# aws-samples/sagemaker-distributed-training-pytorch-kr

Measured on AMD Instinct MI355X. Metric: tokens/sec (whole node) GPT-2 345M pretrain, higher is better.
Workload: dtype bf16; 1 GPU; model=gpt2-345m (24L h1024 16A, vocab 50304), global_batch=64, seq_len=1024, micro_batch=64, grad_accum=1, parallelism=tp1pp1dp1, layout=baseline, tp=1, pp=1, dp=1, flash_attn=True, recompute=none, gemm_autotune=preloaded, comm_stream_priority=high, optimizer_overlap=False, mlp_gelu_fusion=gemm_tn epilogues (fc1 bias+GeLU fwd, fc2 dgrad+GeLU bwd)

## Files before the change

sagemaker-distributed-training-pytorch-kr_amd/csrc/bindings.cpp:

```cpp
#include <torch/extension.h>
#include <c10/hip/HIPStream.h>
#include <c10/hip/HIPGuard.h>

#include "kernels/launchers.h"

namespace {

using torch::Tensor;
using OptT = std::optional<Tensor>;

hipStream_t cur_stream() { return c10::hip::getCurrentHIPStream().stream(); }

int dcode(const Tensor& t) {
  switch (t.scalar_type()) {
    case at::kFloat: return 0;
    case at::kBFloat16: return 1;
    case at::kHalf: return 2;
    default: TORCH_CHECK(false, "smdt_amd: unsupported dtype ", t.scalar_type());
  }
}

void check(hipError_t e, const char* what) {
  TORCH_CHECK(e == hipSuccess, "smdt_amd kernel '", what, "' failed: ", hipGetErrorString(e));
}
// ... 408 lines not shown
  check(smdt_gemm_mx((int)out_dtype, a.scalar_type() == at::kFloat8_e5m2 ? 1 : 0, a.data_ptr(), sa.data_ptr(),
                     b.data_ptr(), sb.data_ptr(), out.data_ptr(), optr(bias), M, N, K, (int)max_blocks, cur_stream()),
        "gemm_mx");
  return out;
}

void fp8_update_scales(Tensor scale, Tensor hist, Tensor amax, Tensor fmt_max, int64_t margin, bool use_max) {
  need_contig(scale, "scale");
  need_contig(hist, "amax_history");
  need_contig(amax, "amax");
  need_contig(fmt_max, "fmt_max");
  TORCH_CHECK(scale.dim() == 1 && hist.dim() == 2 && amax.dim() == 1 && fmt_max.dim() == 1,
              "fp8_update_scales: scale [T], amax_history [T, H], amax [T], fmt_max [T]");
  const int64_t T = scale.size(0), H = hist.size(1);
  TORCH_CHECK(T >= 1 && H >= 1 && hist.size(0) == T && amax.size(0) == T && fmt_max.size(0) == T,
              "fp8_update_scales: table sizes do not match");
  for (const Tensor* t : {&scale, &hist, &amax, &fmt_max})
    TORCH_CHECK(t->scalar_type() == at::kFloat && t->device() == scale.device(), "fp8_update_scales: fp32 tables "
                "on one device");
  TORCH_CHECK(margin >= 0 && margin <= 64, "fp8_update_scales: margin out of range");
  check(smdt_fp8_update_scales(scale.data_ptr<float>(), hist.data_ptr<float>(), amax.data_ptr<float>(),
                               fmt_max.data_ptr<float>(), T, H, (int)margin, use_max ? 1 : 0, cur_stream()),
        "fp8_update_scales");
}

Tensor transpose2d(Tensor x) {
  need_contig(x, "x");
  TORCH_CHECK(x.dim() == 2, "transpose2d: x must be 2-D");
  TORCH_CHECK(x.scalar_type() == at::kBFloat16 || x.scalar_type() == at::kHalf, "transpose2d: bf16 / fp16 only");
  TORCH_CHECK(x.size(0) % 8 == 0 && x.size(1) % 8 == 0, "transpose2d: both dims must be multiples of 8");
  auto out = torch::empty({x.size(1), x.size(0)}, x.options());
  check(smdt_transpose16(x.data_ptr(), out.data_ptr(), x.size(0), x.size(1), cur_stream()), "transpose2d");
  return out;
}

void paced_copy(Tensor recv, Tensor send, int64_t blocks, int64_t ns) {
  need_contig(recv, "recv");
  need_contig(send, "send");
  TORCH_CHECK(recv.is_cuda() && send.is_cuda(), "paced_copy: CUDA tensors");
  const int64_t nb = send.numel() * send.element_size();
  TORCH_CHECK(nb == recv.numel() * recv.element_size() && nb % 16 == 0, "paced_copy: equal sizes, multiple of 16 B");
  TORCH_CHECK((uintptr_t)send.data_ptr() % 16 == 0 && (uintptr_t)recv.data_ptr() % 16 == 0, "paced_copy: 16-B aligned");
  check(smdt_paced_copy(send.data_ptr(), recv.data_ptr(), nb, (int)blocks, ns, cur_stream()), "paced_copy");
}

void rope_(Tensor x, Tensor cos_t, Tensor sin_t, int64_t rot, int64_t pos_div, int64_t pos_mod,
           bool backward) {
  need_cuda(x, "x");
  TORCH_CHECK(x.dim() == 3 && x.stride(2) == 1, "rope: x must be [ntok, nh, d] with unit last stride");
  need_contig(cos_t, "cos");
  need_contig(sin_t, "sin");
  TORCH_CHECK(cos_t.scalar_type() == at::kFloat && sin_t.scalar_type() == at::kFloat, "rope: fp32 tables");
  TORCH_CHECK(rot <= x.size(2) && rot % 16 == 0 && cos_t.size(-1) == rot / 2, "rope: rotary dim mismatch");
  TORCH_CHECK(x.stride(0) % 8 == 0 && x.stride(1) % 8 == 0, "rope: strides must keep 16-byte alignment");
  check(smdt_rope(dcode(x), x.data_ptr(), x.size(0), (int)x.size(1), x.stride(0), x.stride(1),
                  (int)rot, cos_t.data_ptr<float>(), sin_t.data_ptr<float>(), (int)pos_div,
                  (int)pos_mod, backward ? 1 : 0, cur_stream()),
        "rope");
}

bool gemm_tn_supported(Tensor a, Tensor b) {
  if (!a.is_cuda() || !b.is_cuda() || a.dim() != 2 || b.dim() != 2 || !a.is_contiguous() || !b.is_contiguous()) return false;
  if ((a.scalar_type() != at::kBFloat16 && a.scalar_type() != at::kHalf) || b.scalar_type() != a.scalar_type()) return false;
  if (a.size(1) != b.size(1)) return false;
  if (reinterpret_cast<uintptr_t>(a.data_ptr()) % 16 || reinterpret_cast<uintptr_t>(b.data_ptr()) % 16) return false;
  return smdt_gemm_tn_supported(a.size(0), b.size(0), a.size(1)) != 0;
// ... 625 lines not shown
  check(smdt_relay_epoch_bump(s.data(), (int)s.size(), (int)rank, (int)nranks_local, (uint32_t)n, cur_stream()),
        "relay_epoch_bump");
}

}

void register_blaslt(pybind11::module_& m);

PYBIND11_MODULE(TORCH_EXTENSION_NAME, m) {
  m.doc() = "smdt_amd gfx950 (MI355X) HIP kernel library";
  register_blaslt(m);
  using pybind11::arg;
  m.def("layernorm_fwd", &layernorm_fwd, arg("x"), arg("res"), arg("bias"), arg("gamma"), arg("beta"),
        arg("eps"), arg("p_drop"), arg("seed"), arg("offset"), arg("rms"), arg("want_s"),
        arg("out_y") = pybind11::none(), arg("x2") = pybind11::none());
  m.def("layernorm_bwd", &layernorm_bwd, arg("dy"), arg("ds_in"), arg("s"), arg("gamma"), arg("mean"),
        arg("rstd"), arg("p_drop"), arg("seed"), arg("offset"), arg("rms"), arg("want_dx"), arg("want_dbias"),
        arg("dgamma_acc") = pybind11::none(), arg("dbeta_acc") = pybind11::none(),
        arg("dbias_acc") = pybind11::none(), arg("out_dx") = pybind11::none(), arg("dy2") = pybind11::none());
  m.def("bias_act_fwd", &bias_act_fwd);
  m.def("bias_act_bwd", &bias_act_bwd, arg("dy"), arg("x"), arg("bias"), arg("act"), arg("want_dbias"),
        arg("dbias_acc") = pybind11::none());
  m.def("swiglu_fwd", &swiglu_fwd);
  m.def("swiglu_bwd", &swiglu_bwd);
  m.def("softmax_fwd", &softmax_fwd);
  m.def("softmax_bwd", &softmax_bwd);
  m.def("adam", &adam);
  m.def("sumsq", &sumsq);
  m.def("clip_coef", &clip_coef);
  m.def("scale_", &scale_);
  m.def("cast_", &cast_);
  m.def("rope_", &rope_);
  m.def("transpose2d", &transpose2d);
  m.def("fp8_quantize", &fp8_quantize);
  m.def("fp8_update_scales", &fp8_update_scales);
  m.def("mx_quantize", &mx_quantize, arg("x"), arg("fmt"), arg("rows") = true, arg("cols") = false);
  m.def("gemm_mx", &gemm_mx, arg("a"), arg("sa"), arg("b"), arg("sb"), arg("bias") = pybind11::none(),
        arg("out_dtype") = 1, arg("max_blocks") = 0);
  m.def("gemm_mx_supported", &gemm_mx_supported);
  m.def("paced_copy", &paced_copy);
  m.def("gather_rows", &gather_rows);
  m.def("aug_depthwise", &aug_depthwise);
  m.def("aug_median3", &aug_median3);
  m.def("bias_grad", &bias_grad);
  m.def("gemm_tn_supported", &gemm_tn_supported, arg("a"), arg("b"));
  m.def("gemm_tn", &gemm_tn, arg("a"), arg("b"), arg("epi") = 0, arg("bias") = pybind11::none(),
        arg("out") = pybind11::none(), arg("out2") = pybind11::none(), arg("max_blocks") = 0,
        arg("var") = 0, arg("aux") = pybind11::none());
  m.def("wgrad_mfma", &wgrad_mfma, arg("main_grad"), arg("dy"), arg("x"), arg("max_splits") = 0);
  m.def("wgrad_grouped", &wgrad_grouped, arg("main_grads"), arg("dys"), arg("xs"),
        arg("biases") = std::vector<Tensor>{}, arg("overwrite") = std::vector<bool>{}, arg("cus") = 0,
        arg("mranges") = std::vector<Tensor>{}, arg("experts") = std::vector<int64_t>{});
  m.def("moe_rows", [](int64_t T, int64_t E) { return smdt_moe_rows(T, E); });
  m.def("gemm_tn_shape_supported", [](int64_t M, int64_t N, int64_t K) { return smdt_gemm_tn_supported(M, N, K) != 0; });
  m.def("moe_route", &moe_route);
  m.def("moe_route_into", &moe_route_into);
  m.def("ptr_table", &ptr_table);
  m.def("gemm_tn_grouped", &gemm_tn_grouped, arg("a"), arg("btab"), arg("n"), arg("tile_expert"), arg("epi") = 0,
        arg("biastab") = pybind11::none(), arg("aux") = pybind11::none(), arg("sums") = false,
        arg("max_blocks") = 0);
  m.def("wgrad_fp8_grouped", &wgrad_fp8_grouped, arg("main_grads"), arg("dys"), arg("xs"), arg("inv_dys"),
        arg("inv_xs"), arg("overwrite") = std::vector<bool>{}, arg("cus") = 0);
  m.def("wgrad_fp8_supported", &wgrad_fp8_supported);
  m.def("ce_stats", &ce_stats);
  m.def("set_rng_step", &set_rng_step);
  m.def("adam_capturable", &adam_capturable);
// ... 45 lines not shown
```

sagemaker-distributed-training-pytorch-kr_amd/csrc/kernels/launchers.h:

```cpp
#pragma once
#include <hip/hip_runtime.h>
#include <stdint.h>

extern "C" {

int smdt_ln_bwd_nblocks(int64_t rows, int H);
hipError_t smdt_layernorm_fwd(int dtype, int wdtype, const void* x, const void* res,
                              const void* bias, const void* gamma, const void* beta, void* y,
                              void* s_out, float* mean, float* rstd, int64_t rows, int H,
                              float eps, float p_drop, uint64_t seed, uint64_t offset, int rms,
                              const void* x2, hipStream_t st);
hipError_t smdt_layernorm_bwd(int dtype, int wdtype, const void* dy, const void* ds_in,
                              const void* s, const void* gamma, const float* mean,
                              const float* rstd, void* ds_out, void* dx_out, float* partials,
                              int nblocks, float* dgamma, float* dbeta, float* dbias,
                              int64_t rows, int H, float p_drop, uint64_t seed, uint64_t offset,
                              int rms, int acc_mask, const void* dy2, hipStream_t st);

int smdt_bias_act_slices(int64_t rows, int N);
hipError_t smdt_bias_act_fwd(int dtype, int act, const void* x, const void* bias, void* y,
                             int64_t rows, int N, hipStream_t st);
hipError_t smdt_bias_act_bwd(int dtype, int act, const void* dy, const void* x, const void* bias,
                             void* dx, float* partials, float* dbias, int64_t rows, int N,
                             int accumulate, hipStream_t st);
// ... 4 lines not shown
hipError_t smdt_swiglu_fwd(int dtype, const void* x, void* y, int64_t rows, int F,
                           hipStream_t st);
hipError_t smdt_swiglu_bwd(int dtype, const void* dy, const void* x, void* dx, int64_t rows,
                           int F, hipStream_t st);

hipError_t smdt_softmax_fwd(int dtype, int mode, const void* x, const uint8_t* mask, void* y,
                            int64_t rows, int sq, int sk, int heads, float scale,
                            hipStream_t st);
hipError_t smdt_softmax_bwd(int dtype, int mode, const void* dy, const void* y, void* dx,
                            int64_t rows, int sq, int sk, float scale, hipStream_t st);

extern "C" void smdt_set_rng_step(uint32_t* counter);
extern "C" uint32_t* smdt_rng_step();

hipError_t smdt_adam(float* master, const float* grad, float* m, float* v, void* model_out,
                     int model_dtype, int64_t n, float lr, float beta1, float beta2, float eps,
                     float wd, float bc1, float bc2, int adamw, const float* grad_mul,
                     const int* found_inf, const float* hyper, hipStream_t st);
int smdt_sumsq_nblocks(int64_t n);
hipError_t smdt_sumsq(int dtype, const void* x, int64_t n, float* partial, int nblocks,
                      float* out, int* found_inf, hipStream_t st);
hipError_t smdt_clip_coef(const float* sumsq, float max_norm, float inv_scale, float* mul_out,
                          float* norm_out, hipStream_t st);
hipError_t smdt_scale(int dtype, void* x, int64_t n, const float* mul, float cmul,
                      hipStream_t st);
hipError_t smdt_cast(int in_dtype, int out_dtype, const void* x, void* y, int64_t n,
                     int accumulate, hipStream_t st);

hipError_t smdt_rope(int dtype, void* x, int64_t ntok, int nh, int64_t tok_stride,
                     int64_t head_stride, int rot, const float* cos_t, const float* sin_t,
                     int pos_div, int pos_mod, int backward, hipStream_t st);

hipError_t smdt_transpose16(const void* in, void* out, int64_t R, int64_t C, hipStream_t st);
hipError_t smdt_fp8_quantize(const void* x, void* q, void* qt, const float* scale, float* amax, int64_t M,
                             int64_t K, int dtype, int bf8, hipStream_t st);
hipError_t smdt_fp8_update_scales(float* scale, float* hist, float* amax, const float* fmt_max, int64_t T,
                                  int64_t H, int margin, int use_max, hipStream_t st);
hipError_t smdt_mx_quantize(const void* x, void* q, void* s, void* qt, void* st, int64_t R, int64_t C, int dtype,
                            int bf8, hipStream_t st_);
int smdt_gemm_mx_supported(int64_t M, int64_t N, int64_t K);
hipError_t smdt_gemm_mx(int dtype, int a_bf8, const void* a, const void* sa, const void* b, const void* sb, void* c,
                        const void* bias, int64_t M, int64_t N, int64_t K, int max_blocks, hipStream_t st);
hipError_t smdt_paced_copy(const void* src, void* dst, int64_t nbytes, int blocks, int64_t ns, hipStream_t st);
hipError_t smdt_gather_rows(const void* src, const int64_t* map, void* dst, int64_t nrows, int64_t nsrc,
                            int64_t row_bytes, hipStream_t st);

hipError_t smdt_ce_stats(int dtype, const void* logits, const int64_t* target, int64_t rows,
                         int V, int Vvalid, int64_t vstart, float* row_max, float* row_sumexp,
                         float* row_tgt, hipStream_t st);
hipError_t smdt_ce_bwd(int dtype, const void* logits, const int64_t* target, const float* gmax,
                       const float* gsum, const float* dloss, void* dlogits, int64_t rows, int V,
                       int Vvalid, int64_t vstart, int64_t ignore_index, hipStream_t st);
hipError_t smdt_ce_fused(int dtype, void* logits, const int64_t* target, float* loss, int64_t rows,
                         int V, int Vvalid, int64_t ignore_index, int local, int64_t vstart, hipStream_t st);

hipError_t smdt_aug_depthwise(const float* x, const float* k, float* y, int N, int C, int H, int W, int ks,
                              hipStream_t st);
hipError_t smdt_aug_median3(const float* x, float* y, int planes, int H, int W, hipStream_t st);

hipError_t smdt_flash_fwd(int dtype, const void* q, const void* k, const void* v, void* o,
                          float* lse, int B, int H, int Hkv, int S, int D, int64_t q_sb,
                          int64_t q_ss, int64_t q_sh, int64_t k_sb, int64_t k_ss, int64_t k_sh,
                          int64_t v_sb, int64_t v_ss, int64_t v_sh, int64_t o_sb, int64_t o_ss,
                          int64_t o_sh, float scale, int causal, float dropout_p, uint64_t seed,
                          uint64_t offset, hipStream_t st);
hipError_t smdt_flash_bwd(int dtype, const void* q, const void* k, const void* v, const void* o,
// ... 110 lines not shown
```

sagemaker-distributed-training-pytorch-kr_amd/csrc/kernels/transpose.hip:

```cpp
#include "common.h"
#include "launchers.h"

namespace smdt {

constexpr int kTT = 64;

__global__ __launch_bounds__(256) void transpose16_kernel(const uint16_t* __restrict__ in,
                                                          uint16_t* __restrict__ out, int R, int C) {
  __shared__ uint16_t t[kTT][kTT + 2];
  const int r0 = blockIdx.x * kTT, c0 = blockIdx.y * kTT;
#pragma unroll
  for (int k = 0; k < 2; ++k) {
    const int v = threadIdx.x + k * 256;
    const int rr = v >> 3, cv = (v & 7) * 8;
    const int r = r0 + rr, c = c0 + cv;
    if (r < R && c < C) {
      const u16x8 x = __builtin_nontemporal_load(reinterpret_cast<const u16x8*>(in + (int64_t)r * C + c));
#pragma unroll
      for (int j = 0; j < 8; ++j) t[rr][cv + j] = x[j];
    }
  }
  __syncthreads();
#pragma unroll
  for (int k = 0; k < 2; ++k) {
    const int v = threadIdx.x + k * 256;
    const int cc = v >> 3, rv = (v & 7) * 8;
    const int c = c0 + cc, r = r0 + rv;
    if (c < C && r < R) {
      u16x8 y;
#pragma unroll
      for (int j = 0; j < 8; ++j) y[j] = t[rv + j][cc];
      *reinterpret_cast<u16x8*>(out + (int64_t)c * R + r) = y;
    }
  }
}

__global__ __launch_bounds__(512) void gather_rows_kernel(const uint8_t* __restrict__ src,
                                                          const int64_t* __restrict__ map,
                                                          uint8_t* __restrict__ dst, int64_t nrows,
                                                          int64_t nsrc, int64_t rb) {
  const int64_t chunks = (rb + 1023) / 1024;
  const int64_t item = (int64_t)blockIdx.x * 8 + (threadIdx.x >> 6);
  if (item >= nrows * chunks) return;
  const int64_t r = item / chunks;
  const int64_t off = (item - r * chunks) * 1024 + (int64_t)(threadIdx.x & 63) * 16;
  if (off >= rb) return;
  const int64_t s = map[r];
  u16x8 v = {};
  if (s >= 0 && s < nsrc) v = __builtin_nontemporal_load(reinterpret_cast<const u16x8*>(src + s * rb + off));
  *reinterpret_cast<u16x8*>(dst + r * rb + off) = v;
}

}

using namespace smdt;

extern "C" hipError_t smdt_gather_rows(const void* src, const int64_t* map, void* dst, int64_t nrows,
                                       int64_t nsrc, int64_t row_bytes, hipStream_t st) {
  if (nrows <= 0) return hipSuccess;
  if (row_bytes <= 0 || row_bytes % 16 != 0) return hipErrorInvalidValue;
  const int64_t items = nrows * ((row_bytes + 1023) / 1024);
  const int64_t blocks = (items + 7) / 8;
  if (blocks > 0x7FFFFFFF) return hipErrorInvalidValue;
  hipLaunchKernelGGL(gather_rows_kernel, dim3((unsigned)blocks), dim3(512), 0, st, (const uint8_t*)src, map,
                     (uint8_t*)dst, nrows, nsrc, row_bytes);
  return hipGetLastError();
}

extern "C" hipError_t smdt_transpose16(const void* in, void* out, int64_t R, int64_t C, hipStream_t st) {
  if (R <= 0 || C <= 0 || R % 8 != 0 || C % 8 != 0 || R > (1 << 30) || C > (1 << 30))
    return hipErrorInvalidValue;
  const int64_t gx = (R + kTT - 1) / kTT, gy = (C + kTT - 1) / kTT;
  if (gy > 65535) return hipErrorInvalidValue;
  hipLaunchKernelGGL(transpose16_kernel, dim3((unsigned)gx, (unsigned)gy), dim3(256), 0, st,
                     (const uint16_t*)in, (uint16_t*)out, (int)R, (int)C);
  return hipGetLastError();
}
```

sagemaker-distributed-training-pytorch-kr_amd/models/transformer.py:

```python
from __future__ import annotations

import math
import os
from dataclasses import dataclass, field
from typing import Optional

import torch
import torch.nn as nn
import torch.nn.functional as F

from ..ops import _ext
from ..ops import functional as SF
from ..parallel import state as ps
from ..parallel import tensor_parallel as tp
from ..parallel.random import checkpoint as rng_checkpoint, get_rng


@dataclass
class TransformerConfig:
    num_layers: int = 24
    hidden_size: int = 1024
    num_attention_heads: int = 16
    num_query_groups: Optional[int] = None
    ffn_hidden_size: Optional[int] = None
# ... 505 lines not shown
            cfg.params_dtype, device, None, 0, 1))
        self.router_bias = nn.Parameter(torch.zeros(e, dtype=cfg.params_dtype, device=device))
        self.experts = nn.ModuleList(ParallelMLP(cfg, layer_number, device, key=f"layers.{layer_number}.experts.{i}")
                                     for i in range(e))
        self._tabs = None

    def route(self, flat):
        prob = torch.softmax(F.linear(flat, self.router, self.router_bias).float(), dim=-1)
        return prob.max(dim=-1)

    def _grouped_check(self, flat):
        cfg = self.cfg
        why = None
        if ps.get_state().tp > 1:
            why = "tensor parallel size 1"
        elif cfg.activation != "gelu":
            why = f"the gelu activation (got {cfg.activation})"
        elif not cfg.add_bias_linear:
            why = "linear biases (--disable-bias-linear is set)"
        elif cfg.fp8:
            why = "16-bit experts (fp8 is set)"
        kern = _ext.use_kernels(flat)
        if why is None and kern:
            T, h, f, E = flat.shape[0], cfg.hidden_size, cfg.ffn_hidden_size, len(self.experts)
            R = SF.moe_rows(T, E)
            C = _ext.ext()
            probe = self.experts[0]
            if flat.dtype not in (torch.bfloat16, torch.float16) or probe.fc1.weight.dtype != flat.dtype:
                why = f"bf16 or fp16 activations and weights (got {flat.dtype} / {probe.fc1.weight.dtype})"
            elif not (C.gemm_tn_shape_supported(R, f, h) and C.gemm_tn_shape_supported(R, h, f)):
                why = (f"gemm_tn shapes: hidden {h} and ffn {f} multiples of 256 (rows {R})")
            elif torch.is_grad_enabled() and any(
                    getattr(p, "main_grad", None) is None or p.main_grad.dtype != torch.float32
                    or isinstance(getattr(type(p), "main_grad", None), property)
                    for ex in self.experts for p in (ex.fc1.weight, ex.fc1.bias, ex.fc2.weight, ex.fc2.bias)):
                why = "a plain fp32 main_grad on every expert weight and bias (a DDP wrapper with fp32 gradients)"
        if why is not None:
            raise RuntimeError(f"--moe-grouped-gemm needs {why}")
        return kern

    def _forward_grouped(self, x):
        s, b, h = x.shape
        flat = x.reshape(s * b, h)
        kern = self._grouped_check(flat)
        logits = F.linear(flat, self.router, self.router_bias)
        route = SF.moe_route(logits)
        self.last_counts = route[6]
        top_p = torch.softmax(logits.float(), dim=-1).gather(1, route[1].long().unsqueeze(1)).squeeze(1)
        ex = self.experts
        w1, b1 = [e.fc1.weight for e in ex], [e.fc1.bias for e in ex]
        w2, b2 = [e.fc2.weight for e in ex], [e.fc2.bias for e in ex]
        tabs = None
        if kern:
            key = tuple(p.data_ptr() for p in w1 + b1 + w2 + b2)
            if self._tabs is None or self._tabs[0] != key:
                self._tabs = (key, (SF.moe_pointer_tables(w1, b1), SF.moe_pointer_tables(w2, b2)))
            tabs = self._tabs[1]
        out = tp.GroupedSwitchExperts.apply(flat, top_p, route, tabs, len(ex), *w1, *b1, *w2, *b2)
        return out.view(s, b, h), None

    def forward(self, x):
        if self.cfg.moe_grouped_gemm:
            return self._forward_grouped(x)
        s, b, h = x.shape
        flat = x.reshape(s * b, h)
        top_p, top_e = self.route(flat)
        order = torch.argsort(top_e, stable=True)
# ... 179 lines not shown
```

sagemaker-distributed-training-pytorch-kr_amd/optim/optimizer.py:

```python
from __future__ import annotations

import math
import os
from typing import Optional

import torch
import torch.distributed as dist

from ..comm import health as _health
from ..comm import stats as _cs
from ..ops import _ext
from ..parallel import state as ps
from ..parallel.distributed import DistributedDataParallel
from ..parallel import tensor_parallel as _tp


class DynamicLossScaler:

    def __init__(self, initial_scale=2.0 ** 32, min_scale=1.0, growth_factor=2.0, backoff_factor=0.5,
                 growth_interval=1000, hysteresis=2, device=None):
        self.scale = torch.tensor([float(initial_scale)], dtype=torch.float32, device=device)
        self.min_scale = float(min_scale)
        self.growth_factor, self.backoff_factor = growth_factor, backoff_factor
        self.growth_interval = int(growth_interval)
# ... 211 lines not shown
        if gr.dtype != torch.float32:
            gr = gr.float()
        if use_k:
            model_out = None if self.param_is_fp32 else ddp.param_data[s:e]
            host_out = None
            if model_out is not None and not model_out.is_cuda:
                host_out, model_out = model_out, torch.empty(n, dtype=model_out.dtype, device=mst.device)
            if self.capturable:
                _ext.ext().adam_capturable(mst, gr, m, v, model_out, self._hyp, self.beta1, self.beta2,
                                           self.eps, wd, self.adamw, mul, self.found_inf)
            else:
                _ext.ext().adam(mst, gr, m, v, model_out, self.lr, self.beta1, self.beta2, self.eps, wd, t,
                                self.adamw, mul, self.found_inf)
            if host_out is not None:
                host_out.copy_(model_out)
            if self.param_is_fp32:
                ddp.param_data[s:e].copy_(mst)
        else:
            ok = (self.found_inf == 0).float()
            gg = torch.where(self.found_inf == 0, gr * mul, torch.zeros_like(gr))
            if not self.adamw and wd:
                gg = gg + wd * mst
            m.mul_(1 - (1 - self.beta1) * ok).add_(gg * ((1 - self.beta1) * ok))
            v.mul_(1 - (1 - self.beta2) * ok).add_(gg * gg * ((1 - self.beta2) * ok))
            denom = v.sqrt() / math.sqrt(bc2) + self.eps
            upd = (m / bc1) / denom
            if self.adamw and wd:
                upd = upd + wd * mst
            mst.sub_(self.lr * upd * ok)
            ddp.param_data[s:e].copy_(mst.to(ddp.param_data.dtype))

    def _step_overlapped(self, g, mul, t):
        ddp = self.ddp
        cur = torch.cuda.current_stream(self.device)
        if getattr(self, "_opt_stream", None) is None:
            self._opt_stream = torch.cuda.Stream(device=self.device)
        side = self._opt_stream
        side.wait_stream(cur)
        delay = int(os.environ.get("SMDT_OPT_STREAM_DELAY", "0"))
        with torch.cuda.stream(side):
            for i in ddp.opt_bucket_order:
                if delay:
                    torch.cuda._sleep(delay)
                s, e, key = self.pieces[i]
                if e <= s:
                    continue
                mo, n = self.master_off[i], e - s
                wd = self.weight_decay if key[0] else 0.0
                gr = g[s:e]
                _ext.ext().adam(self.master[mo:mo + n], gr, self.exp_avg[mo:mo + n], self.exp_avg_sq[mo:mo + n],
                                ddp.param_data[s:e], self.lr, self.beta1, self.beta2, self.eps, wd, t, self.adamw,
                                mul, self.found_inf)
                gr.zero_()
                ev = torch.cuda.Event()
                ev.record(side)
                ddp._opt_events[i] = ev
        mul.record_stream(side)
        ddp._async_zeroed = True

    @torch.no_grad()
    def repair_params(self):
        _tp.params_changed()
        ddp = self.ddp
        if hasattr(ddp, "wait_param_gather"):
            ddp.wait_param_gather()
        for (s, e, _), mo in zip(self.pieces, self.master_off):
# ... 74 lines not shown
```

sagemaker-distributed-training-pytorch-kr_amd/parallel/distributed.py:

```python
from __future__ import annotations

import contextlib
import os
from dataclasses import dataclass, field
from typing import Dict, List, Optional, Tuple

import torch
import torch.distributed as dist
import torch.nn as nn

from ..comm import buckets as _buckets
from ..comm import health as _health
from ..comm import stats as _cs
from ..ops import _ext
from . import state as ps
from . import zero_init as _zi


@dataclass
class Bucket:
    index: int
    region: tuple
    start: int
    end: int
# ... 93 lines not shown
            cur: Optional[Bucket] = None
            for p in regions[key]:
                n = _zi.logical_numel(p)
                alone = bool(getattr(p, "shared_embedding", False)) and st.pp > 1
                if cur is not None and cur.params and (alone or cur.alone):
                    cur.end = _round_up(off, align)
                    off = cur.end
                    cur = None
                if cur is None or (off - cur.start + n > bucket_size and cur.params):
                    if cur is not None:
                        cur.end = _round_up(off, align)
                        off = cur.end
                    cur = Bucket(len(self.buckets), key, off, off, alone=alone)
                    self.buckets.append(cur)
                self.param_index[id(p)] = (off, n)
                cur.params.append(p)
                self.param_bucket[id(p)] = cur
                off += _round_up(n, 16)
            if cur is not None:
                cur.end = _round_up(off, align)
                off = cur.end
        self.numel = off
        self.params = params
        self.param_data = torch.zeros(0 if self._zero_init else self.numel, dtype=pdtype, device=dev)
        self.shapes = {id(p): ((_zi.logical_shape(p), _contig_strides(_zi.logical_shape(p)))
                               if _zi.is_partitioned(p) else (tuple(p.shape), tuple(p.stride()))) for p in params}
        self.grad_store = None
        self.zero3 = None
        self._staging: Dict[int, torch.Tensor] = {}
        self._rs_inflight: Dict[int, tuple] = {}
        self._direct = self.zero_stage >= 2 and self.dp == 1
        self._lazy_zero = (self.zero_stage >= 2 and not self._direct
                           and os.environ.get("SMDT_LAZY_GRAD_ZERO", "1") == "1")
        self._fresh: Dict[int, set] = {}
        self._claimed: set = set()
        self._gaps: Dict[int, list] = {}
        if self.zero_stage >= 2:
            off = 0
            for b in self.buckets:
                b.shard_off = off
                off += b.numel // self.dp
            self.grad_store = torch.zeros(off, dtype=grad_dtype, device=dev)
            self.grad_data = ShardedFlat(self, self.grad_store)
            self._store_fresh = set(range(len(self.buckets)))
        else:
            self.grad_data = torch.zeros(self.numel, dtype=grad_dtype, device=dev)
        with torch.no_grad():
            for p in params:
                o, n = self.param_index[id(p)]
                if not self._zero_init:
                    pv = _dense_view(self.param_data[o:o + n], p)
                    pv.copy_(p.data)
                    p.data = pv
                if self.zero_stage >= 2:
                    _make_lazy_grad_param(p, self)
                else:
                    p.main_grad = _dense_view(self.grad_data[o:o + n], p)
                p._smdt_grad_ready = self._on_grad_ready
        self._hooks = [p.register_post_accumulate_grad_hook(self._post_accumulate) for p in params]
        self.regions = self._region_ranges()
        self.overlap_param_gather = bool(overlap_param_gather and use_distributed_optimizer and self.dp > 1)
        self._pg_hooks = []
        if self.overlap_param_gather:
            for mod in module.modules():
                own = [p for p in mod._parameters.values() if p is not None and id(p) in self.param_bucket]
                if own:
                    bks = sorted({self.param_bucket[id(p)].index for p in own})
                    self._pg_hooks.append(mod.register_forward_pre_hook(self._make_gather_wait(bks)))
        self._opt_events: Dict[int, object] = {}
        self._async_zeroed = False
        self.overlap_optimizer = bool(use_distributed_optimizer and self.dp == 1 and dev.type == "cuda"
                                      and st.pp == 1 and not torch_compat
                                      and os.environ.get("SMDT_OVERLAP_OPTIMIZER", "1") == "1")
        self.opt_bucket_order = list(reversed(range(len(self.buckets))))
        if self.overlap_optimizer:
            self._install_update_waits(module)
        self._reset_pending()
        if self.dp > 1 and not self._zero_init:
            self.broadcast_params()

    def _region_ranges(self):
        out = {}
        for b in self.buckets:
            s, e = out.get(b.region, (b.start, b.end))
            out[b.region] = (min(s, b.start), max(e, b.end))
        return out

    def shard_range(self, b: Bucket) -> Tuple[int, int]:
        sz = b.numel // self.dp
        s = b.start + self.dp_rank * sz
        return s, s + sz
# ... 32 lines not shown
        b = self.param_bucket.get(id(p))
        if b is not None and self.zero_stage >= 2:
            left = b.pending.get(id(p), 0) - 1
            if left > 0:
                b.pending[id(p)] = left
                return
            b.pending.pop(id(p), None)
            if self._direct and not b.pending:
                b.pending = {id(q): int(getattr(q, "_smdt_grad_contributions", 1)) for q in b.params}
            elif self.overlap and not b.pending and b.index in self._staging:
                self._launch(b)
            return
        if b is None or not self.sync_enabled:
            return
        left = b.pending.get(id(p), 0) - 1
        if left > 0:
            b.pending[id(p)] = left
            return
        b.pending.pop(id(p), None)
        if self.sync_enabled and self.overlap and not b.pending and not b.launched:
            self._launch(b)

    def _reset_pending(self):
        for b in self.buckets:
            b.pending = {id(p): int(getattr(p, "_smdt_grad_contributions", 1)) for p in b.params}
            b.launched = False
            b.handle = None

    def _launch(self, b: Bucket):
        b.launched = True
        if self.zero_stage >= 2:
            self._launch_sharded(b)
            return
        if self.dp == 1:
            return
        view = self.grad_data[b.start:b.end]
        nb = view.numel() * view.element_size()
        if self.deterministic:
            folded = self._fold(view)
            if self.zero:
                s, e = self.shard_range(b)
                self.grad_data[s:e].copy_(folded[s - b.start:e - b.start])
            else:
                view.copy_(folded)
            b.handle = None
            return
        if self.zero:
            s, e = self.shard_range(b)
            out = self.grad_data[s:e]
            h = self._xg().reduce_scatter_async(out, view, op="avg") if self._xg() is not None else None
            if h is not None:
                b.handle = h
                _cs.collective("reduce_scatter", self.dp_group, nb, transport="xgmi", events=h.timing())
                return
            if self.use_avg:
                b.handle = dist.reduce_scatter_tensor(out, view, op=dist.ReduceOp.AVG, group=self.dp_group,
                                                      async_op=True)
            else:
                view.div_(self.dp)
                b.handle = dist.reduce_scatter_tensor(out, view, group=self.dp_group, async_op=True)
            _cs.collective("reduce_scatter", self.dp_group, nb, work=b.handle)
        else:
            h = self._xg().all_reduce_async(view, op="avg") if self._xg() is not None else None
            if h is not None:
                b.handle = h
                _cs.collective("all_reduce", self.dp_group, nb, transport="xgmi", events=h.timing())
                return
            if self.use_avg:
                b.handle = dist.all_reduce(view, op=dist.ReduceOp.AVG, group=self.dp_group, async_op=True)
            else:
                view.div_(self.dp)
                b.handle = dist.all_reduce(view, group=self.dp_group, async_op=True)
            _cs.collective("all_reduce", self.dp_group, nb, work=b.handle)

    def bucket_at(self, i: int) -> Bucket:
        import bisect
        if not hasattr(self, "_starts"):
            self._starts = [b.start for b in self.buckets]
        return self.buckets[bisect.bisect_right(self._starts, i) - 1]

    def _main_grad(self, p) -> torch.Tensor:
        v = self._mg_raw(p)
        if self._lazy_zero:
            fr = self._fresh.get(self.param_bucket[id(p)].index)
            if fr is not None and id(p) in fr:
                fr.discard(id(p))
                v.zero_()
            elif id(p) in self._claimed:
                from .tensor_parallel import flush_deferred_wgrad
                flush_deferred_wgrad()
                self._claimed.clear()
        return v

    def _mg_raw(self, p) -> torch.Tensor:
        b = self.param_bucket[id(p)]
        if self._direct:
            o, n = self.param_index[id(p)]
            shape, stride = self.shapes[id(p)]
            flat = self.grad_store[b.shard_off + (o - b.start):b.shard_off + (o - b.start) + n]
            return flat.view(shape) if _is_dense(shape, stride) else flat.as_strided(shape, stride)
        buf = self._staging.get(b.index)
        if buf is None:
            buf = self._new_staging(b)
        o, n = self.param_index[id(p)]
        shape, stride = self.shapes[id(p)]
        flat = buf[o - b.start:o - b.start + n]
        return flat.view(shape) if _is_dense(shape, stride) else flat.as_strided(shape, stride)

    def _mg_claim(self, p) -> bool:
        if not self._lazy_zero:
            return False
        fr = self._fresh.get(self.param_bucket[id(p)].index)
        if fr is None or id(p) not in fr:
            return False
        fr.discard(id(p))
        self._claimed.add(id(p))
        return True

    def _new_staging(self, b: Bucket) -> torch.Tensor:
        dev = self.grad_store.device
        if not self._lazy_zero:
            buf = torch.zeros(b.numel, dtype=self.grad_dtype, device=dev)
        else:
            buf = torch.empty(b.numel, dtype=self.grad_dtype, device=dev)
            gaps = self._gaps.get(b.index)
            if gaps is None:
                spans = sorted((o - b.start, o - b.start + n) for o, n in (self.param_index[id(q)] for q in b.params))
# ... 140 lines not shown
                    if b.region[2]:
                        g = self.bucket_shard_grad(b)
                        with _cs.blocking("all_reduce", st.tp_group, g.numel() * g.element_size()):
                            dist.all_reduce(g, group=st.tp_group)
            self._reset_pending()
            if self.zero3 is not None:
                self.zero3.end_of_backward()
            return
        self.start_grad_sync()
        for b in self.buckets:
            if b.handle is not None:
                b.handle.wait()
        self._check_xgmi()
        st = self.st
        if st.tp > 1 and st.tp_group is not None:
            for key, (s, e) in self.regions.items():
                if key[2]:
                    with _cs.blocking("all_reduce", st.tp_group, (e - s) * self.grad_data.element_size()):
                        dist.all_reduce(self.grad_data[s:e], group=st.tp_group)
        self._reset_pending()

    def _check_xgmi(self):
        self._syncs += 1
        if torch.cuda.is_available() and torch.cuda.is_current_stream_capturing():
            return
        _health.monitor().launch()

    def zero_grad_buffer(self):
        _health.monitor().consume()
        if self.xgmi is not None and not self.xgmi.active:
            self.xgmi = None
        if self._async_zeroed:
            self._async_zeroed = False
        elif self._direct:
            self.grad_store.zero_()
        elif self.zero_stage >= 2:
            for b in self.buckets:
                self._retire_rs(b)
            self._staging.clear()
            self._fresh.clear()
            self._claimed.clear()
            self._store_fresh = set(range(len(self.buckets)))
        else:
            self.grad_data.zero_()
        for p in self.params:
            p.grad = None
        self._reset_pending()

    def grad_memory_numel(self) -> int:
        return self.grad_store.numel() if self.grad_store is not None else self.grad_data.numel()

    @torch.no_grad()
    def broadcast_params(self):
        src = dist.get_global_rank(self.dp_group, 0) if self.dp > 1 else dist.get_rank()
        dist.broadcast(self.param_data, src=src, group=self.dp_group)

    @torch.no_grad()
    def all_gather_params(self):
        if self.zero3 is not None:
            self.zero3.after_step()
            return
        if self.dp == 1:
            return
        self.wait_param_gather()
        for b in reversed(self.buckets):
            s, e = self.shard_range(b)
            full, mine = self.param_data[b.start:b.end], self.param_data[s:e]
            h = self._xg().all_gather_async(full, mine) if self._xg() is not None else None
            nb = full.numel() * full.element_size()
            if h is not None:
                b.ag_handle = h
                _cs.collective("all_gather", self.dp_group, nb, transport="xgmi", events=h.timing())
            else:
                b.ag_handle = dist.all_gather_into_tensor(full, mine, group=self.dp_group, async_op=True)
                _cs.collective("all_gather", self.dp_group, nb, work=b.ag_handle)
        if not self.overlap_param_gather:
            self.wait_param_gather()

    def wait_param_gather(self, indices=None):
        if self._opt_events:
            self.wait_param_update(indices)
        for b in (self.buckets if indices is None else (self.buckets[i] for i in indices)):
            h = getattr(b, "ag_handle", None)
            if h is not None:
                with _cs.waiting("dp"):
                    h.wait()
                b.ag_handle = None

    def wait_param_update(self, indices=None):
        cur = torch.cuda.current_stream(self.param_data.device) if self._opt_events else None
        for i in (list(self._opt_events) if indices is None else indices):
# ... 124 lines not shown
```

sagemaker-distributed-training-pytorch-kr_amd/parallel/tensor_parallel.py:

```python
from __future__ import annotations

import contextlib
import hashlib
import math
import os
import weakref
from typing import Optional

import torch
import torch.distributed as dist
import torch.nn as nn
import torch.nn.functional as F

from ..comm import loopback as _lb
from ..comm import relay as _relay
from ..comm import stats as _cs
from ..ops import _ext
from ..ops import functional as SF
from . import state as ps



def _tp_size():
    return ps.get_state().tp
# ... 299 lines not shown
            raise ValueError("deferred wgrad: a ranged item takes 16-bit operands and an accumulating target")
        if (scales is not None) != (g2.dtype in _FP8_DTYPES) or (scales is not None and bias is not None):
            raise ValueError("deferred wgrad: FP8 operands come with scales=(inv_dy, inv_x) and no bias, "
                             "16-bit operands without scales")
        if self.hold_bytes_cap is None:
            self.hold_bytes_cap = self._hold_cap(g2.device)
        key = mg.data_ptr()
        g2, t2 = g2.contiguous(), t2.contiguous()
        seg = (g2, t2, g2._version, t2._version)
        nbytes = g2.numel() * g2.element_size() + t2.numel() * t2.element_size()
        it = self.by_key.get(key)
        if it is not None and (mrange is not None or it[8] is not None):
            self.flush()
            it = None
        if it is not None and (it[3] or self.hold or self.merge_repeats):
            it[2].append(seg)
            it[4] = it[4] or not self.hold
        else:
            if it is not None:
                self.flush()
            it = [weight, mg, [seg], self.hold and mrange is None, not self.hold or mrange is not None, bias,
                  bool(fresh), scales, mrange]
            self.items.append(it)
            self.by_key[key] = it
            self.tiles += -(-g2.shape[1] // 256) * -(-t2.shape[1] // 256)
        self.held_bytes += nbytes
        if self.held_bytes > self.hold_bytes_cap:
            self.flush()
        elif not self.hold and not self.defer:
            ready = [x for x in self.items if x[4]]
            tiles = sum(-(-x[2][0][0].shape[1] // 256) * -(-x[2][0][1].shape[1] // 256) for x in ready)
            if tiles >= self.flush_tiles or len(ready) >= 32:
                self.flush(complete_only=True)

    def flush_opportunistic(self):
        if not self.defer:
            self.flush()

    @torch.no_grad()
    def flush(self, complete_only: bool = False):
        if not self.items:
            return
        if complete_only:
            items = [it for it in self.items if it[4]]
            keep = [it for it in self.items if not it[4]]
        else:
            items, keep = self.items, []
        if not items:
            return
        self.items = keep
        self.by_key = {it[1].data_ptr(): it for it in keep}
        self.tiles = sum(-(-it[2][0][0].shape[1] // 256) * -(-it[2][0][1].shape[1] // 256) for it in keep)
        self.held_bytes = sum(sg[0].numel() * sg[0].element_size() + sg[1].numel() * sg[1].element_size()
                              for it in keep for sg in it[2])
        work = []
        for weight, mg, segs, _held, complete, bias, fresh, scales, mrange in items:
            for g2, t2, vg, vt in segs:
                if g2._version != vg or t2._version != vt:
                    raise RuntimeError("deferred wgrad: a queued dY / X tensor was modified in place before the "
                                       "flush; disable with SMDT_DEFER_WGRAD=0 and report the op that did it")
            if len(segs) == 1:
                work.append((weight, mg, [(segs[0][0], segs[0][1])], complete, bias, fresh, scales, mrange))
            elif self.concat_segments and _held:
                work.append((weight, mg, [(_cat_rows([sg[0] for sg in segs]), _cat_rows([sg[1] for sg in segs]))],
                             complete, bias, fresh, scales, mrange))
            else:
# ... 329 lines not shown

def _wgrad_and_bias(weight, bias_p, g2, t2):
    if bias_p is not None and _WGRAD_BIAS and g2.is_cuda:
        raw = getattr(weight, "_smdt_mg_raw", None)
        mg = raw() if raw is not None else getattr(weight, "main_grad", None)
        tgt = SF.grad_accumulate_target(bias_p)
        if mg is not None and tgt is not None and tgt.numel() == g2.shape[-1] and DEFERRED_WGRAD.eligible(mg, g2, t2):
            DEFERRED_WGRAD.push(weight, mg, g2, t2, bias=bias_p,
                                fresh=raw is not None and weight._smdt_mg_claim())
            return None, None
    dw = _wgrad(weight, g2, t2)
    return dw, (_bias_grad(bias_p, g2) if bias_p is not None else None)


_DGRAD_TN = os.environ.get("SMDT_DGRAD_TN", "1") == "1"


_WT_CACHE_ON = os.environ.get("SMDT_DGRAD_WT_CACHE", "1") == "1"
_WT_CACHE: dict = {}


def params_changed():
    _WT_CACHE.clear()
    _PARAMS_EPOCH[0] += 1
    for s in list(_FP8_STATES):
        s._wq.clear()
    _MX_WQ.clear()


def drop_cached_weight_t(params):
    _PARAMS_EPOCH[0] += 1
    for p in params:
        _WT_CACHE.pop(id(p), None)
        for s in list(_FP8_STATES):
            s._wq.pop(id(p), None)
        _MX_WQ.pop(id(p), None)


def mm_rows(g, w):
    M = g.numel() // g.shape[-1]
    bl = _row_blocks(M) if g.is_cuda else None
    if bl is None:
        return g.matmul(w)
    g2 = g.reshape(M, g.shape[-1])
    out = g.new_empty(tuple(g.shape[:-1]) + (w.shape[1],))
    o2 = out.view(M, w.shape[1])
    for a, b in bl:
        torch.mm(g2[a:b], w, out=o2[a:b])
    return out


def _dgrad_weight_t(weight):
    if (_DGRAD_TN and weight.is_cuda and weight.dim() == 2 and weight.is_contiguous()
            and weight.dtype in (torch.bfloat16, torch.float16)
            and weight.shape[0] % 8 == 0 and weight.shape[1] % 8 == 0
            and _ext.use_kernels(weight)):
        if not _WT_CACHE_ON:
            return _ext.ext().transpose2d(weight)
        key = (weight.data_ptr(), weight._version, tuple(weight.shape), weight.dtype)
        hit = _WT_CACHE.get(id(weight))
        if hit is not None and hit[0] == key:
            return hit[1]
        wt = _ext.ext().transpose2d(weight)
        _WT_CACHE[id(weight)] = (key, wt)
        return wt
    return None


_ROW_SPLIT = int(os.environ.get("SMDT_GEMM_ROW_SPLIT", "4096"))


def _row_blocks(M: int):
    q = _ROW_SPLIT
    if q <= 0 or M <= q:
        return None
    r = M % q
    if r == 0 or r > q // 6:
        return None
    return ((0, M - r), (M - r, M))


_GEMM_TN = os.environ.get("SMDT_GEMM_TN", "0")


def _gemm_tn_shapes():
    if _GEMM_TN in ("0", "", "1"):
        return None
    out = set()
    for item in _GEMM_TN.split(","):
        n, k = item.split(":")
        out.add((int(n), int(k)))
    return out


_GEMM_TN_SHAPES = _gemm_tn_shapes()
# ... 1634 lines not shown
```

Baseline: 415,000 tokens/s.

## Batch per-step weight transposes into one kernel and lazily zero flat grads

Adds a table-driven batched transpose kernel. When the parameter epoch changes, the first dgrad weight-transpose request transposes every weight seen in the previous step in a single launch into one flat buffer, instead of one launch per weight. Separately, the DDP flat gradient buffer gets a lazy-zero path for 2-D params: their zeroing is skipped when a deferred wgrad store will overwrite them, and only eager ranges are zeroed at zero_grad. This removes per-weight launch overhead and a large memset, at the cost of extra bookkeeping and a persistent transposed-weight buffer.

```diff
diff --git a/sagemaker-distributed-training-pytorch-kr_amd/csrc/bindings.cpp b/sagemaker-distributed-training-pytorch-kr_amd/csrc/bindings.cpp
--- a/sagemaker-distributed-training-pytorch-kr_amd/csrc/bindings.cpp
+++ b/sagemaker-distributed-training-pytorch-kr_amd/csrc/bindings.cpp
@@ -464,6 +464,45 @@
   auto out = torch::empty({x.size(1), x.size(0)}, x.options());
   check(smdt_transpose16(x.data_ptr(), out.data_ptr(), x.size(0), x.size(1), cur_stream()), "transpose2d");
   return out;
+}
+
+std::tuple<Tensor, int64_t> transpose2d_table(std::vector<Tensor> srcs, std::vector<Tensor> dsts) {
+  const size_t n = srcs.size();
+  TORCH_CHECK(n > 0 && dsts.size() == n && n < (1u << 20), "transpose2d_table: srcs / dsts list lengths");
+  std::vector<const void*> sp(n);
+  std::vector<void*> dp(n);
+  std::vector<int64_t> rows(n), cols(n);
+  for (size_t i = 0; i < n; ++i) {
+    const Tensor &x = srcs[i], &y = dsts[i];
+    need_contig(x, "src");
+    need_contig(y, "dst");
+    TORCH_CHECK(x.is_cuda() && y.is_cuda() && x.device() == srcs[0].device() && y.device() == x.device(),
+                "transpose2d_table: CUDA tensors on one device");
+    TORCH_CHECK(x.dim() == 2 && y.dim() == 2 && y.size(0) == x.size(1) && y.size(1) == x.size(0),
+                "transpose2d_table: dst must be [cols, rows] of its src");
+    TORCH_CHECK((x.scalar_type() == at::kBFloat16 || x.scalar_type() == at::kHalf) && y.scalar_type() == x.scalar_type(),
+                "transpose2d_table: bf16 / fp16 only, dst typed like src");
+    TORCH_CHECK(x.size(0) % 8 == 0 && x.size(1) % 8 == 0, "transpose2d_table: both dims must be multiples of 8");
+    sp[i] = x.data_ptr();
+    dp[i] = y.data_ptr();
+    rows[i] = x.size(0);
+    cols[i] = x.size(1);
+  }
+  Tensor host = torch::empty({(int64_t)(n * sizeof(SmdtTransposeEntry))}, torch::dtype(torch::kUInt8));
+  int64_t tiles = 0;
+  check(smdt_transpose16_table(sp.data(), dp.data(), rows.data(), cols.data(), (int)n,
+                               reinterpret_cast<SmdtTransposeEntry*>(host.data_ptr()), &tiles), "transpose2d_table");
+  return {host.to(srcs[0].device()), tiles};
+}
+
+void transpose2d_batched(Tensor table, int64_t tiles) {
+  need_contig(table, "table");
+  TORCH_CHECK(table.is_cuda() && table.scalar_type() == at::kByte && table.numel() > 0 &&
+              table.numel() % (int64_t)sizeof(SmdtTransposeEntry) == 0, "transpose2d_batched: not a transpose2d_table");
+  const int64_t n = table.numel() / (int64_t)sizeof(SmdtTransposeEntry);
+  TORCH_CHECK(tiles >= n && tiles <= 0x7FFFFFFF, "transpose2d_batched: tile count does not fit the table");
+  check(smdt_transpose16_batched(reinterpret_cast<const SmdtTransposeEntry*>(table.data_ptr()), (int)n, tiles,
+                                 cur_stream()), "transpose2d_batched");
 }
 
 void paced_copy(Tensor recv, Tensor send, int64_t blocks, int64_t ns) {
@@ -1155,6 +1194,8 @@
   m.def("cast_", &cast_);
   m.def("rope_", &rope_);
   m.def("transpose2d", &transpose2d);
+  m.def("transpose2d_table", &transpose2d_table);
+  m.def("transpose2d_batched", &transpose2d_batched);
   m.def("fp8_quantize", &fp8_quantize);
   m.def("fp8_update_scales", &fp8_update_scales);
   m.def("mx_quantize", &mx_quantize, arg("x"), arg("fmt"), arg("rows") = true, arg("cols") = false);
diff --git a/sagemaker-distributed-training-pytorch-kr_amd/csrc/kernels/launchers.h b/sagemaker-distributed-training-pytorch-kr_amd/csrc/kernels/launchers.h
--- a/sagemaker-distributed-training-pytorch-kr_amd/csrc/kernels/launchers.h
+++ b/sagemaker-distributed-training-pytorch-kr_amd/csrc/kernels/launchers.h
@@ -60,6 +60,16 @@
                      int pos_div, int pos_mod, int backward, hipStream_t st);
 
 hipError_t smdt_transpose16(const void* in, void* out, int64_t R, int64_t C, hipStream_t st);
+struct SmdtTransposeEntry {
+  const void* src;
+  void* dst;
+  int rows, cols;
+  int first_tile;
+  int tiles_c;
+};
+hipError_t smdt_transpose16_table(const void* const* srcs, void* const* dsts, const int64_t* rows,
+                                  const int64_t* cols, int n, SmdtTransposeEntry* tab, int64_t* tiles);
+hipError_t smdt_transpose16_batched(const SmdtTransposeEntry* tab, int n, int64_t tiles, hipStream_t st);
 hipError_t smdt_fp8_quantize(const void* x, void* q, void* qt, const float* scale, float* amax, int64_t M,
                              int64_t K, int dtype, int bf8, hipStream_t st);
 hipError_t smdt_fp8_update_scales(float* scale, float* hist, float* amax, const float* fmt_max, int64_t T,
diff --git a/sagemaker-distributed-training-pytorch-kr_amd/csrc/kernels/transpose.hip b/sagemaker-distributed-training-pytorch-kr_amd/csrc/kernels/transpose.hip
--- a/sagemaker-distributed-training-pytorch-kr_amd/csrc/kernels/transpose.hip
+++ b/sagemaker-distributed-training-pytorch-kr_amd/csrc/kernels/transpose.hip
@@ -5,10 +5,8 @@
 
 constexpr int kTT = 64;
 
-__global__ __launch_bounds__(256) void transpose16_kernel(const uint16_t* __restrict__ in,
-                                                          uint16_t* __restrict__ out, int R, int C) {
-  __shared__ uint16_t t[kTT][kTT + 2];
-  const int r0 = blockIdx.x * kTT, c0 = blockIdx.y * kTT;
+__device__ __forceinline__ void transpose16_tile(const uint16_t* __restrict__ in, uint16_t* __restrict__ out,
+                                                 int R, int C, int r0, int c0, uint16_t (*t)[kTT + 2]) {
 #pragma unroll
   for (int k = 0; k < 2; ++k) {
     const int v = threadIdx.x + k * 256;
@@ -33,6 +31,28 @@
       *reinterpret_cast<u16x8*>(out + (int64_t)c * R + r) = y;
     }
   }
+}
+
+__global__ __launch_bounds__(256) void transpose16_kernel(const uint16_t* __restrict__ in,
+                                                          uint16_t* __restrict__ out, int R, int C) {
+  __shared__ uint16_t t[kTT][kTT + 2];
+  transpose16_tile(in, out, R, C, blockIdx.x * kTT, blockIdx.y * kTT, t);
+}
+
+__global__ __launch_bounds__(256) void transpose16_batched_kernel(const SmdtTransposeEntry* __restrict__ tab,
+                                                                  int n) {
+  __shared__ uint16_t t[kTT][kTT + 2];
+  const int b = blockIdx.x;
+  int lo = 0, hi = n - 1;
+  while (lo < hi) {
+    const int mid = (lo + hi + 1) >> 1;
+    if (tab[mid].first_tile <= b) lo = mid; else hi = mid - 1;
+  }
+  const SmdtTransposeEntry e = tab[lo];
+  const int local = b - e.first_tile;
+  const int tr = local / e.tiles_c, tc = local - tr * e.tiles_c;
+  if (tr * kTT >= e.rows) return;
+  transpose16_tile((const uint16_t*)e.src, (uint16_t*)e.dst, e.rows, e.cols, tr * kTT, tc * kTT, t);
 }
 
 __global__ __launch_bounds__(512) void gather_rows_kernel(const uint8_t* __restrict__ src,
@@ -76,3 +96,27 @@
                      (const uint16_t*)in, (uint16_t*)out, (int)R, (int)C);
   return hipGetLastError();
 }
+
+extern "C" hipError_t smdt_transpose16_table(const void* const* srcs, void* const* dsts, const int64_t* rows,
+                                             const int64_t* cols, int n, SmdtTransposeEntry* tab, int64_t* tiles) {
+  if (n <= 0) return hipErrorInvalidValue;
+  int64_t first = 0;
+  for (int i = 0; i < n; ++i) {
+    const int64_t R = rows[i], C = cols[i];
+    if (R <= 0 || C <= 0 || R % 8 != 0 || C % 8 != 0 || R > (1 << 30) || C > (1 << 30) || !srcs[i] || !dsts[i])
+      return hipErrorInvalidValue;
+    if (((uintptr_t)srcs[i] | (uintptr_t)dsts[i]) & 15) return hipErrorInvalidValue;
+    const int64_t tr = (R + kTT - 1) / kTT, tc = (C + kTT - 1) / kTT;
+    tab[i] = SmdtTransposeEntry{srcs[i], dsts[i], (int)R, (int)C, (int)first, (int)tc};
+    first += tr * tc;
+    if (first > 0x7FFFFFFF) return hipErrorInvalidValue;
+  }
+  *tiles = first;
+  return hipSuccess;
+}
+
+extern "C" hipError_t smdt_transpose16_batched(const SmdtTransposeEntry* tab, int n, int64_t tiles, hipStream_t st) {
+  if (!tab || n <= 0 || tiles <= 0 || tiles > 0x7FFFFFFF) return hipErrorInvalidValue;
+  hipLaunchKernelGGL(transpose16_batched_kernel, dim3((unsigned)tiles), dim3(256), 0, st, tab, n);
+  return hipGetLastError();
+}
diff --git a/sagemaker-distributed-training-pytorch-kr_amd/models/transformer.py b/sagemaker-distributed-training-pytorch-kr_amd/models/transformer.py
--- a/sagemaker-distributed-training-pytorch-kr_amd/models/transformer.py
+++ b/sagemaker-distributed-training-pytorch-kr_amd/models/transformer.py
@@ -561,7 +561,7 @@
                 why = (f"gemm_tn shapes: hidden {h} and ffn {f} multiples of 256 (rows {R})")
             elif torch.is_grad_enabled() and any(
                     getattr(p, "main_grad", None) is None or p.main_grad.dtype != torch.float32
-                    or isinstance(getattr(type(p), "main_grad", None), property)
+                    or getattr(getattr(p, "_smdt_ddp", None), "zero_stage", 0) >= 2
                     for ex in self.experts for p in (ex.fc1.weight, ex.fc1.bias, ex.fc2.weight, ex.fc2.bias)):
                 why = "a plain fp32 main_grad on every expert weight and bias (a DDP wrapper with fp32 gradients)"
         if why is not None:
diff --git a/sagemaker-distributed-training-pytorch-kr_amd/optim/optimizer.py b/sagemaker-distributed-training-pytorch-kr_amd/optim/optimizer.py
--- a/sagemaker-distributed-training-pytorch-kr_amd/optim/optimizer.py
+++ b/sagemaker-distributed-training-pytorch-kr_amd/optim/optimizer.py
@@ -267,6 +267,7 @@
 
     def _step_overlapped(self, g, mul, t):
         ddp = self.ddp
+        _tp.params_in_flight()
         cur = torch.cuda.current_stream(self.device)
         if getattr(self, "_opt_stream", None) is None:
             self._opt_stream = torch.cuda.Stream(device=self.device)
diff --git a/sagemaker-distributed-training-pytorch-kr_amd/parallel/distributed.py b/sagemaker-distributed-training-pytorch-kr_amd/parallel/distributed.py
--- a/sagemaker-distributed-training-pytorch-kr_amd/parallel/distributed.py
+++ b/sagemaker-distributed-training-pytorch-kr_amd/parallel/distributed.py
@@ -149,6 +149,12 @@
         self._direct = self.zero_stage >= 2 and self.dp == 1
         self._lazy_zero = (self.zero_stage >= 2 and not self._direct
                            and os.environ.get("SMDT_LAZY_GRAD_ZERO", "1") == "1")
+        from .tensor_parallel import STORE_GRAD_BATCH_WT
+        self._lazy_flat = (self.zero_stage < 2 and not torch_compat and grad_dtype == torch.float32
+                           and not self._zero_init and STORE_GRAD_BATCH_WT)
+        self._lazy_zero = self._lazy_zero or self._lazy_flat
+        self._flat_views: Dict[int, torch.Tensor] = {}
+        self._eager: List[Tuple[int, int]] = []
         self._fresh: Dict[int, set] = {}
         self._claimed: set = set()
         self._gaps: Dict[int, list] = {}
@@ -171,9 +177,20 @@
                     p.data = pv
                 if self.zero_stage >= 2:
                     _make_lazy_grad_param(p, self)
+                elif self._lazy_flat and p.dim() >= 2 and type(p) in (nn.Parameter, _LazyGradParameter):
+                    self._flat_views[id(p)] = _dense_view(self.grad_data[o:o + n], p)
+                    _make_lazy_grad_param(p, self)
                 else:
+                    if type(p) is _LazyGradParameter:
+                        p.__class__ = nn.Parameter
                     p.main_grad = _dense_view(self.grad_data[o:o + n], p)
                 p._smdt_grad_ready = self._on_grad_ready
+        if self._lazy_flat:
+            joined = False
+            for o, n, lazy in sorted((*self.param_index[id(p)], id(p) in self._flat_views) for p in params):
+                if not lazy:
+                    self._eager.append((self._eager.pop()[0] if joined else o, o + n))
+                joined = not lazy
         self._hooks = [p.register_post_accumulate_grad_hook(self._post_accumulate) for p in params]
         self.regions = self._region_ranges()
         self.overlap_param_gather = bool(overlap_param_gather and use_distributed_optimizer and self.dp > 1)
@@ -272,22 +289,24 @@
         if self.zero_stage >= 2:
             self._launch_sharded(b)
             return
+        if self._lazy_flat:
+            self._zero_unwritten(b, self._grad_flat[b.start:b.end])
         if self.dp == 1:
             return
-        view = self.grad_data[b.start:b.end]
+        view = self._grad_flat[b.start:b.end]
         nb = view.numel() * view.element_size()
         if self.deterministic:
             folded = self._fold(view)
             if self.zero:
                 s, e = self.shard_range(b)
-                self.grad_data[s:e].copy_(folded[s - b.start:e - b.start])
+                self._grad_flat[s:e].copy_(folded[s - b.start:e - b.start])
             else:
                 view.copy_(folded)
             b.handle = None
             return
         if self.zero:
             s, e = self.shard_range(b)
-            out = self.grad_data[s:e]
+            out = self._grad_flat[s:e]
             h = self._xg().reduce_scatter_async(out, view, op="avg") if self._xg() is not None else None
             if h is not None:
                 b.handle = h
@@ -326,6 +345,11 @@
             if fr is not None and id(p) in fr:
                 fr.discard(id(p))
                 v.zero_()
+            elif id(p) in self._claimed and self._lazy_flat:
+                from .tensor_parallel import DEFERRED_WGRAD
+                self._claimed.discard(id(p))
+                if DEFERRED_WGRAD.revoke_store(v):
+                    v.zero_()
             elif id(p) in self._claimed:
                 from .tensor_parallel import flush_deferred_wgrad
                 flush_deferred_wgrad()
@@ -333,6 +357,8 @@
         return v
 
     def _mg_raw(self, p) -> torch.Tensor:
+        if self._lazy_flat:
+            return self._flat_views[id(p)]
         b = self.param_bucket[id(p)]
         if self._direct:
             o, n = self.param_index[id(p)]
@@ -539,6 +565,14 @@
             self.xgmi = None
         if self._async_zeroed:
             self._async_zeroed = False
+            if self._lazy_flat:
+                self._fresh.clear()
+                self._claimed.clear()
+        elif self._lazy_flat:
+            for lo, hi in self._eager:
+                self._grad_flat[lo:hi].zero_()
+            self._fresh = {b.index: {id(q) for q in b.params if id(q) in self._flat_views} for b in self.buckets}
+            self._claimed.clear()
         elif self._direct:
             self.grad_store.zero_()
         elif self.zero_stage >= 2:
@@ -554,6 +588,25 @@
             p.grad = None
         self._reset_pending()
 
+    @property
+    def grad_data(self):
+        if self._lazy_flat and (self._fresh or self._claimed):
+            self._materialize()
+        return self._grad_flat
+
+    @grad_data.setter
+    def grad_data(self, v):
+        self._grad_flat = v
+
+    def _materialize(self):
+        from .tensor_parallel import DEFERRED_WGRAD
+        for b in self.buckets:
+            self._zero_unwritten(b, self._grad_flat[b.start:b.end])
+        for i in self._claimed:
+            if DEFERRED_WGRAD.revoke_store(self._flat_views[i]):
+                self._flat_views[i].zero_()
+        self._claimed.clear()
+
     def grad_memory_numel(self) -> int:
         return self.grad_store.numel() if self.grad_store is not None else self.grad_data.numel()
 
@@ -564,6 +617,9 @@
 
     @torch.no_grad()
     def all_gather_params(self):
+        if self.zero3 is not None or (self.dp > 1 and self.overlap_param_gather):
+            from .tensor_parallel import params_in_flight
+            params_in_flight()
         if self.zero3 is not None:
             self.zero3.after_step()
             return
diff --git a/sagemaker-distributed-training-pytorch-kr_amd/parallel/tensor_parallel.py b/sagemaker-distributed-training-pytorch-kr_amd/parallel/tensor_parallel.py
--- a/sagemaker-distributed-training-pytorch-kr_amd/parallel/tensor_parallel.py
+++ b/sagemaker-distributed-training-pytorch-kr_amd/parallel/tensor_parallel.py
@@ -355,6 +355,13 @@
             tiles = sum(-(-x[2][0][0].shape[1] // 256) * -(-x[2][0][1].shape[1] // 256) for x in ready)
             if tiles >= self.flush_tiles or len(ready) >= 32:
                 self.flush(complete_only=True)
+
+    def revoke_store(self, mg) -> bool:
+        it = self.by_key.get(mg.data_ptr())
+        if it is None or not it[6]:
+            return False
+        it[6] = False
+        return True
 
     def flush_opportunistic(self):
         if not self.defer:
@@ -750,9 +757,72 @@
     _PARAMS_EPOCH[0] += 1
     for p in params:
         _WT_CACHE.pop(id(p), None)
+        _WT_BATCH.forget(id(p))
         for s in list(_FP8_STATES):
             s._wq.pop(id(p), None)
         _MX_WQ.pop(id(p), None)
+
+
+def params_in_flight():
+    _WT_BATCH.skip_epoch = _PARAMS_EPOCH[0]
+
+
+STORE_GRAD_BATCH_WT = os.environ.get("SMDT_STORE_GRAD_BATCH_WT", "1") == "1"
+
+
+class _WeightTBatch:
+
+    def __init__(self):
+        self.epoch = -1
+        self.skip_epoch = -1
+        self.prev = {}
+        self.cur = {}
+        self.sig = None
+        self.table = None
+        self.launches = 0
+
+    def forget(self, pid):
+        self.prev.pop(pid, None)
+        self.cur.pop(pid, None)
+
+    def request(self, weight):
+        ep = _PARAMS_EPOCH[0]
+        if ep != self.epoch:
+            self.epoch = ep
+            self.prev, self.cur = self.cur, {}
+            if self.skip_epoch != ep:
+                self._refresh(weight.device)
+        self.cur[id(weight)] = weakref.ref(weight)
+
+    def _refresh(self, dev):
+        ws = []
+        for r in self.prev.values():
+            w = r()
+            if (w is not None and w.device == dev and w.dim() == 2 and w.is_contiguous() and w.numel() > 0
+                    and w.dtype in (torch.bfloat16, torch.float16)
+                    and w.shape[0] % 8 == 0 and w.shape[1] % 8 == 0 and w.data_ptr() % 16 == 0):
+                ws.append(w)
+        if not ws:
+            return
+        sig = tuple((id(w), w.data_ptr(), tuple(w.shape), w.dtype) for w in ws)
+        if sig != self.sig:
+            if torch.cuda.is_current_stream_capturing():
+                return
+            flat = torch.empty(sum(w.numel() for w in ws), dtype=torch.int16, device=dev)
+            wts, off = [], 0
+            for w in ws:
+                wts.append(flat[off:off + w.numel()].view(w.dtype).view(w.shape[1], w.shape[0]))
+                off += w.numel()
+            table, tiles = _ext.ext().transpose2d_table([w.detach() for w in ws], wts)
+            self.sig, self.table = sig, (table, tiles, wts, flat)
+        table, tiles, wts, _ = self.table
+        _ext.ext().transpose2d_batched(table, tiles)
+        self.launches += 1
+        for w, wt in zip(ws, wts):
+            _WT_CACHE[id(w)] = ((w.data_ptr(), w._version, tuple(w.shape), w.dtype), wt)
+
+
+_WT_BATCH = _WeightTBatch()
 
 
 def mm_rows(g, w):
@@ -778,7 +848,14 @@
         key = (weight.data_ptr(), weight._version, tuple(weight.shape), weight.dtype)
         hit = _WT_CACHE.get(id(weight))
         if hit is not None and hit[0] == key:
+            if STORE_GRAD_BATCH_WT and id(weight) not in _WT_BATCH.cur:
+                _WT_BATCH.cur[id(weight)] = weakref.ref(weight)
             return hit[1]
+        if STORE_GRAD_BATCH_WT:
+            _WT_BATCH.request(weight)
+            hit = _WT_CACHE.get(id(weight))
+            if hit is not None and hit[0] == key:
+                return hit[1]
         wt = _ext.ext().transpose2d(weight)
         _WT_CACHE[id(weight)] = (key, wt)
         return wt
```

New measurement: 415,700 tokens/s, median of 6. Within noise of the previous version (+0.2%).
